# apache/incubator-predictionio

Measured on AMD Instinct MI355X. Metric: als_ratings_per_sec, higher is better.
Workload: dtype fp32; 1 GPU; model=als_rank64_implicit, global_batch=250000000, users=12500000, items=10000000, parallelism=dp1

## Files before the change

### predictionio_amd/ops/csrc/als_kernels.hip

```cpp

#include <hip/hip_runtime.h>

#define CHUNK 16

__device__ __forceinline__ void wave_sync() {
  __builtin_amdgcn_wave_barrier();
}

typedef __attribute__((ext_vector_type(4))) float f32x4_t;
typedef __attribute__((ext_vector_type(2))) float f32x2_t;
typedef __attribute__((ext_vector_type(16))) float f32x16_t;

__device__ __forceinline__ f32x2_t fma2(f32x2_t a, f32x2_t b, f32x2_t c) {
  return __builtin_elementwise_fma(a, b, c);
}

__device__ __forceinline__ int uniform_i32(int v) {
  return __builtin_amdgcn_readfirstlane(v);
}
__device__ __forceinline__ long long uniform_i64(long long v) {
  const unsigned int lo = (unsigned int)uniform_i32((int)(unsigned long long)v);
  const unsigned int hi =
      (unsigned int)uniform_i32((int)((unsigned long long)v >> 32));
  return (long long)(((unsigned long long)hi << 32) | lo);
}
__device__ __forceinline__ float lane_bcast(float v, int k) {
  return __int_as_float(__builtin_amdgcn_readlane(__float_as_int(v), k));
}


template <int F>
__global__ __launch_bounds__(256) void als_solve_kernel(
    const long long* __restrict__ indptr,
    const int* __restrict__ indices,
    const float* __restrict__ values,
    const float* __restrict__ Y,
    const float* __restrict__ YtY,
    float* __restrict__ X,
    int n_rows,
    float lambda,
    float alpha,
    int implicit_mode,
    int wr_scale,
    int skip_below)
{
  constexpr int TM = 4;
  constexpr int TILES = (F / TM) * (F / TM);
  constexpr int TPT = (TILES + 255) / 256;
  constexpr int NB = 16;
  static_assert(F % TM == 0, "F must be divisible by 4");
  static_assert(F % NB == 0, "F must be divisible by the panel width");

  __shared__ float ys[CHUNK][F + 1];
  __shared__ float ws_a[CHUNK];
  __shared__ float ws_b[CHUNK];
  __shared__ float As[F][F + 4];
  __shared__ float bs[F];
  __shared__ float dinv_all[F];

  const int tid = threadIdx.x;
  const int lane = tid & 63;
  const int wave = tid >> 6;

  for (long long row = blockIdx.x; row < n_rows; row += gridDim.x) {
    const long long start = indptr[row];
    const long long end = indptr[row + 1];
    const int nnz = (int)(end - start);
    if (nnz <= skip_below) continue;

    float acc[TPT][TM][TM];
#pragma unroll
    for (int t = 0; t < TPT; ++t)
#pragma unroll
      for (int i = 0; i < TM; ++i)
#pragma unroll
        for (int j = 0; j < TM; ++j) acc[t][i][j] = 0.f;

    for (int i = tid; i < F; i += 256) bs[i] = 0.f;

    for (int base = 0; base < nnz; base += CHUNK) {
      const int cn = min(CHUNK, nnz - base);
      __syncthreads();
      for (int e = tid; e < cn * F; e += 256) {
        const int c = e / F;
        const int k = e % F;
        const int col = indices[start + base + c];
        ys[c][k] = Y[(long long)col * F + k];
      }
      if (tid < cn) {
        const float r = values[start + base + tid];
        if (implicit_mode) {
          ws_a[tid] = alpha * r;
          ws_b[tid] = 1.f + alpha * r;
        } else {
          ws_a[tid] = 1.f;
          ws_b[tid] = r;
        }
      }
      __syncthreads();

      if (tid < F) {
        float bacc = 0.f;
        for (int c = 0; c < cn; ++c) bacc += ws_b[c] * ys[c][tid];
        bs[tid] += bacc;
      }

#pragma unroll
      for (int t = 0; t < TPT; ++t) {
        const int tile = tid + t * 256;
        if (TILES >= 256 || tile < TILES) {
          const int ti = (tile / (F / TM)) * TM;
          const int tj = (tile % (F / TM)) * TM;
          for (int c = 0; c < cn; ++c) {
            const float w = ws_a[c];
            float ya[TM], yb[TM];
#pragma unroll
            for (int i = 0; i < TM; ++i) ya[i] = ys[c][ti + i];
#pragma unroll
            for (int j = 0; j < TM; ++j) yb[j] = ys[c][tj + j];
#pragma unroll
            for (int i = 0; i < TM; ++i)
#pragma unroll
              for (int j = 0; j < TM; ++j)
                acc[t][i][j] = fmaf(w * ya[i], yb[j], acc[t][i][j]);
          }
        }
      }
    }
    __syncthreads();

#pragma unroll
    for (int t = 0; t < TPT; ++t) {
      const int tile = tid + t * 256;
      if (TILES >= 256 || tile < TILES) {
        const int ti = (tile / (F / TM)) * TM;
        const int tj = (tile % (F / TM)) * TM;
#pragma unroll
        for (int i = 0; i < TM; ++i)
#pragma unroll
          for (int j = 0; j < TM; ++j) {
            float v = acc[t][i][j];
            if (YtY != nullptr) v += YtY[(ti + i) * F + (tj + j)];
            As[ti + i][tj + j] = v;
          }
      }
    }
    __syncthreads();
    if (tid < F) {
      const float reg = wr_scale ? lambda * (float)nnz : lambda;
      As[tid][tid] += reg;
    }
    __syncthreads();

    for (int k0 = 0; k0 < F; k0 += NB) {
      if (wave == 0) {
        for (int kk = 0; kk < NB; ++kk) {
          const int kq = k0 + kk;
          wave_sync();
          float d = As[kq][kq];
          d = d > 0.f ? sqrtf(d) : 1e-20f;
          const float dinv = 1.f / d;
          if (lane == kk) {
            As[kq][kq] = d;
            dinv_all[kq] = dinv;
          }
          if (lane > kk && lane < NB) As[k0 + lane][kq] *= dinv;
          wave_sync();
          if (lane > kk && lane < NB) {
            const float lik = As[k0 + lane][kq];
            for (int j = kk + 1; j <= lane; ++j)
              As[k0 + lane][k0 + j] =
                  fmaf(-lik, As[k0 + j][kq], As[k0 + lane][k0 + j]);
          }
        }
      }
      __syncthreads();
      if (k0 + NB >= F) break;
      for (int i = k0 + NB + tid; i < F; i += 256) {
        float w[NB];
#pragma unroll
        for (int m = 0; m < NB; ++m) w[m] = As[i][k0 + m];
#pragma unroll
        for (int j = 0; j < NB; ++j) {
          float s = w[j];
#pragma unroll
          for (int m = 0; m < NB; ++m)
            if (m < j) s = fmaf(-w[m], As[k0 + j][k0 + m], s);
          w[j] = s * dinv_all[k0 + j];
        }
#pragma unroll
        for (int m = 0; m < NB; ++m) As[i][k0 + m] = w[m];
      }
      __syncthreads();
      const int rem = F - k0 - NB;
      const int remt = rem >> 1;
      for (int e = tid; e < remt * remt; e += 256) {
        const int i = k0 + NB + 2 * (e / remt);
        const int j = k0 + NB + 2 * (e % remt);
        if (j <= i) {
          float s00 = As[i][j];
          float s01 = As[i][j + 1];
          float s10 = As[i + 1][j];
          float s11 = As[i + 1][j + 1];
#pragma unroll
          for (int m = 0; m < NB; m += 4) {
            const f32x4_t a0 =
                *reinterpret_cast<const f32x4_t*>(&As[i][k0 + m]);
            const f32x4_t a1 =
                *reinterpret_cast<const f32x4_t*>(&As[i + 1][k0 + m]);
            const f32x4_t b0 =
                *reinterpret_cast<const f32x4_t*>(&As[j][k0 + m]);
            const f32x4_t b1 =
                *reinterpret_cast<const f32x4_t*>(&As[j + 1][k0 + m]);
#pragma unroll
            for (int q = 0; q < 4; ++q) {
              s00 = fmaf(-a0[q], b0[q], s00);
              s01 = fmaf(-a0[q], b1[q], s01);
              s10 = fmaf(-a1[q], b0[q], s10);
              s11 = fmaf(-a1[q], b1[q], s11);
            }
          }
          As[i][j] = s00;
          if (j + 1 <= i) As[i][j + 1] = s01;
          As[i + 1][j] = s10;
          As[i + 1][j + 1] = s11;
        }
      }
      __syncthreads();
    }

    for (int k0 = 0; k0 < F; k0 += NB) {
      if (wave == 0) {
        for (int kk = 0; kk < NB; ++kk) {
          wave_sync();
          const float zk = bs[k0 + kk] * dinv_all[k0 + kk];
          if (lane == kk) bs[k0 + kk] = zk;
          if (lane > kk && lane < NB)
            bs[k0 + lane] = fmaf(-As[k0 + lane][k0 + kk], zk,
                                 bs[k0 + lane]);
        }
      }
      __syncthreads();
      for (int j = k0 + NB + tid; j < F; j += 256) {
        float s = bs[j];
#pragma unroll
        for (int m = 0; m < NB; ++m)
          s = fmaf(-As[j][k0 + m], bs[k0 + m], s);
        bs[j] = s;
      }
      __syncthreads();
    }
    for (int k0 = F - NB; k0 >= 0; k0 -= NB) {
      if (wave == 0) {
        for (int kk = NB - 1; kk >= 0; --kk) {
          wave_sync();
          const float xk = bs[k0 + kk] * dinv_all[k0 + kk];
          if (lane == kk) bs[k0 + kk] = xk;
          if (lane < kk)
            bs[k0 + lane] = fmaf(-As[k0 + kk][k0 + lane], xk,
                                 bs[k0 + lane]);
        }
      }
      __syncthreads();
      for (int j = tid; j < k0; j += 256) {
        float s = bs[j];
#pragma unroll
        for (int m = 0; m < NB; ++m)
          s = fmaf(-As[k0 + m][j], bs[k0 + m], s);
        bs[j] = s;
      }
      __syncthreads();
    }

    if (tid < F) X[row * (long long)F + tid] = bs[tid];
    __syncthreads();
  }
}


constexpr int wave_kernel_min_waves(int f) {
  return f <= 16 ? 6 : (f <= 32 ? 4 : 2);
}

template <int F, bool BF16G = false>
__global__ __launch_bounds__(128, wave_kernel_min_waves(F))
void als_solve_wave_kernel(
    const long long* __restrict__ indptr,
    const int* __restrict__ indices,
    const float* __restrict__ values,
    const float* __restrict__ Y,
    const float* __restrict__ YtY,
    float* __restrict__ X,
    int n_rows,
    float lambda,
    float alpha,
    int implicit_mode,
    int wr_scale,
    int skip_below,
    int skip_above)
{
  static_assert(F <= 64, "wave kernel supports rank <= 64");
  static_assert(!BF16G || F == 64, "MFMA Gramian variant needs F=64");
  const int lane = threadIdx.x & 63;
  const int wave = uniform_i32((int)(threadIdx.x >> 6));

  constexpr int PD = 4;
  constexpr int LP = F + 4;
  __shared__ float ys[2][PD][F];
  constexpr int TP = 40;
  __shared__ unsigned short ysT[2][BF16G ? F : 1][BF16G ? TP : 1];
  __shared__ float Lc[2][F][LP];

  for (long long row = (long long)blockIdx.x * 2 + wave; row < n_rows;
       row += (long long)gridDim.x * 2) {
    const long long start = uniform_i64(indptr[row]);
    const int nnz = uniform_i32((int)(indptr[row + 1] - start));
    if (nnz <= skip_below || nnz > skip_above)
      continue;

    const int ln = lane | (int)(start >> 63);

    f32x2_t ap[F / 2];
#pragma unroll
    for (int m = 0; m < F / 2; ++m) ap[m] = f32x2_t{0.f, 0.f};
    float b_reg = 0.f;

    if constexpr (BF16G) {
      typedef __attribute__((ext_vector_type(8))) unsigned short bf16x8g;
      typedef __attribute__((ext_vector_type(4))) float f32x4g;
      const int lg = lane >> 4;
      const int lq = lane & 15;
      f32x4g accm[4][4];
#pragma unroll
      for (int ti = 0; ti < 4; ++ti)
#pragma unroll
        for (int tj = 0; tj < 4; ++tj)
          accm[ti][tj] = f32x4g{0.f, 0.f, 0.f, 0.f};
      float yn2[PD], wa2[PD], wb2[PD];
#pragma unroll
      for (int p = 0; p < PD; ++p) {
        if (p < nnz) {
          const int col = indices[start + p];
          yn2[p] = lane < F ? Y[(long long)col * F + lane] : 0.f;
          const float v = values[start + p];
          wa2[p] = implicit_mode ? alpha * v : 1.f;
          wb2[p] = implicit_mode ? 1.f + alpha * v : v;
        }
      }
      for (int c0 = 0; c0 < nnz; c0 += 32) {
        for (int cm = 0; cm < 32; ++cm) {
          const int c = c0 + cm;
          const int slot = c & (PD - 1);
          float sy = 0.f;
          if (c < nnz) {
            const float wa = wa2[slot];
            const float sc = sqrtf(wa > 1e-12f ? wa : 1e-12f);
            const float ycur = yn2[slot];
            sy = sc * ycur;
            b_reg = fmaf(wb2[slot], ycur, b_reg);
            if (c + PD < nnz) {
              const int ncol = indices[start + c + PD];
              yn2[slot] = lane < F ? Y[(long long)ncol * F + lane] : 0.f;
              const float nv = values[start + c + PD];
              wa2[slot] = implicit_mode ? alpha * nv : 1.f;
              wb2[slot] = implicit_mode ? 1.f + alpha * nv : nv;
            }
          }
          const unsigned short hb =
              (unsigned short)(__float_as_uint(sy) >> 16);
          const int gcol = (((cm >> 3) ^ (lane & 3)) << 3) | (cm & 7);
          ysT[wave][lane][gcol] = hb;
        }
        wave_sync();
        bf16x8g frag[4];
#pragma unroll
        for (int t = 0; t < 4; ++t) {
          const int row = t * 16 + lq;
          const int g = lg ^ (row & 3);
          frag[t] = *reinterpret_cast<const bf16x8g*>(
              &ysT[wave][row][g << 3]);
        }
#pragma unroll
        for (int ti = 0; ti < 4; ++ti)
#pragma unroll
          for (int tj = 0; tj < 4; ++tj)
            accm[ti][tj] = __builtin_amdgcn_mfma_f32_16x16x32_bf16(
                frag[ti], frag[tj], accm[ti][tj], 0, 0, 0);
        wave_sync();
      }
#pragma unroll
      for (int ti = 0; ti < 4; ++ti)
#pragma unroll
        for (int tj = 0; tj < 4; ++tj)
#pragma unroll
          for (int r = 0; r < 4; ++r)
            Lc[wave][ti * 16 + lg * 4 + r][tj * 16 + lq] =
                accm[ti][tj][r];
      wave_sync();
#pragma unroll
      for (int m = 0; m < F; ++m) ap[m >> 1][m & 1] = Lc[wave][m][lane];
      wave_sync();
    } else {
    float yn[PD], vn[PD];
#pragma unroll
    for (int p = 0; p < PD; ++p) {
      if (p < nnz) {
        const int col = indices[start + p];
        yn[p] = lane < F ? Y[(long long)col * F + lane] : 0.f;
        vn[p] = values[start + p];
      }
    }
    for (int c0 = 0; c0 < nnz; c0 += PD) {
#pragma unroll
      for (int p = 0; p < PD; ++p) {
        const int c = c0 + p;
        if (c >= nnz) break;
        const float ycur = yn[p];
        const float vcur = vn[p];
        if (lane < F) ys[wave][p][lane] = ycur;
        wave_sync();
        if (c + PD < nnz) {
          const int ncol = indices[start + c + PD];
          if (lane < F) yn[p] = Y[(long long)ncol * F + lane];
          vn[p] = values[start + c + PD];
        }
        float w_a, w_b;
        if (implicit_mode) {
          w_a = alpha * vcur;
          w_b = 1.f + alpha * vcur;
        } else {
          w_a = 1.f;
          w_b = vcur;
        }
        b_reg = fmaf(w_b, ycur, b_reg);
        const float wyj = w_a * ycur;
        const f32x2_t wyj2 = {wyj, wyj};
#pragma unroll
        for (int q = 0; q < F / 4; ++q) {
          const f32x4_t y4 =
              *reinterpret_cast<const f32x4_t*>(&ys[wave][p][4 * q]);
          ap[2 * q + 0] = fma2(wyj2, y4.lo, ap[2 * q + 0]);
          ap[2 * q + 1] = fma2(wyj2, y4.hi, ap[2 * q + 1]);
        }
        wave_sync();
      }
    }

    }

    if (YtY != nullptr && lane < F) {
#pragma unroll
      for (int q = 0; q < F / 4; ++q) {
        const f32x4_t t4 = *reinterpret_cast<const f32x4_t*>(
            &YtY[(long long)lane * F + 4 * q]);
        ap[2 * q + 0] += t4.lo;
        ap[2 * q + 1] += t4.hi;
      }
    }
    {
      const float reg = wr_scale ? lambda * (float)nnz : lambda;
#pragma unroll
      for (int m = 0; m < F; ++m)
        if (m == ln) ap[m >> 1][m & 1] += reg;
    }

    float dl = 0.f;
#pragma unroll
    for (int k = 0; k < F; ++k) {
      float lkk = lane_bcast(ap[k >> 1][k & 1], k);
      lkk = lkk > 1e-30f ? lkk : 1e-30f;
      const float dinv = rsqrtf(lkk);
      const float ljk = ln > k ? ap[k >> 1][k & 1] * dinv : 0.f;
      dl = ln == k ? dinv : dl;
      Lc[wave][k][lane < F ? lane : F] = ljk;
      ap[k >> 1][k & 1] = ljk;
      wave_sync();
      const f32x2_t nl2 = {-ljk, -ljk};
#pragma unroll
      for (int m4 = (k + 1) & ~3; m4 < F; m4 += 4) {
        const f32x4_t lq =
            *reinterpret_cast<const f32x4_t*>(&Lc[wave][k][m4]);
        const f32x2_t lh[2] = {lq.lo, lq.hi};
#pragma unroll
        for (int h = 0; h < 2; ++h) {
          const int m2 = m4 + 2 * h;
          if (m2 > k)
            ap[m2 >> 1] = fma2(nl2, lh[h], ap[m2 >> 1]);
          else if (m2 == k)
            ap[m2 >> 1][1] = fmaf(-ljk, lh[h][1], ap[m2 >> 1][1]);
        }
      }
      wave_sync();
    }

#pragma unroll
    for (int k = 0; k < F; ++k) {
      const float zk = lane_bcast(b_reg * dl, k);
      b_reg = fmaf(-ap[k >> 1][k & 1], zk, b_reg);
    }
    b_reg *= dl;
    {
      float4 lq = {0.f, 0.f, 0.f, 0.f};
#pragma unroll
      for (int k = F - 1; k >= 0; --k) {
        if ((k & 3) == 3 && lane < F)
          lq = *reinterpret_cast<const float4*>(&Lc[wave][lane][k & ~3]);
        const float xk = lane_bcast(b_reg * dl, k);
        const float lv = (k & 3) == 0 ? lq.x
                         : (k & 3) == 1 ? lq.y
                         : (k & 3) == 2 ? lq.z : lq.w;
        b_reg = fmaf(ln < k ? -lv : 0.f, xk, b_reg);
      }
      b_reg *= dl;
    }

    if (lane < F) X[row * (long long)F + lane] = b_reg;
  }
}


#define WOODBURY_MAX_NNZ 32


template <int F, int NW, int NLO, bool BF16S = false>
__global__ __launch_bounds__(128, NW > 24 ? 5 : 6) void als_woodbury_kernel(
    const long long* __restrict__ indptr,
    const int* __restrict__ indices,
    const float* __restrict__ values,
    const float* __restrict__ Y,
    const float* __restrict__ V,
    float* __restrict__ X,
    int n_rows,
    float lambda,
    float alpha,
    int implicit_mode,
    int wr_scale,
    unsigned long long* prof)
{
  constexpr int FP = F + 4;
  constexpr int FPH = F + 8;
  const int lane = threadIdx.x & 63;
  const int wave = uniform_i32((int)(threadIdx.x >> 6));

  __shared__ float Yl[2][NW][BF16S ? (FPH / 2) : FP];
  constexpr int MP = NW + 4;
  __shared__ float M[2][NW][MP];
  __shared__ float tv[2][NW];
  __shared__ __attribute__((aligned(16)))
  float dv[2][NW];

  float* yl = &Yl[wave][0][0];
  unsigned short* ylh = reinterpret_cast<unsigned short*>(yl);
  const float* src = implicit_mode ? V : Y;
  const unsigned short* srch = reinterpret_cast<const unsigned short*>(V);

  for (long long row = (long long)blockIdx.x * 2 + wave; row < n_rows;
       row += (long long)gridDim.x * 2) {
    const long long start = uniform_i64(indptr[row]);
    const int n = uniform_i32((int)(indptr[row + 1] - start));
    if (n > NW || n <= NLO) continue;
    if (n == 0 && NLO < 0) {
      for (int e = lane; e < F; e += 64)
        X[row * (long long)F + e] = 0.f;
      continue;
    }
    const bool probe = prof != nullptr && (row & 1023) == 0 && lane == 0;
    unsigned long long pt0 = 0, pt1 = 0, pt2 = 0, pt3 = 0;
    if (probe) pt0 = wall_clock64();

    if (lane < n)
      tv[wave][lane] = __int_as_float(indices[start + lane]);
    wave_sync();
    for (int c = 0; c < n; ++c) {
      const long long col = __float_as_int(tv[wave][c]);
      if constexpr (BF16S) {
        const unsigned int* srow = reinterpret_cast<const unsigned int*>(
            srch + col * F);
        unsigned int* drow =
            reinterpret_cast<unsigned int*>(ylh + c * FPH);
        for (int e = lane; e < F / 2; e += 64) drow[e] = srow[e];
      } else {
        for (int e = lane; e < F; e += 64)
          yl[c * FP + e] = src[col * F + e];
      }
    }
    if (lane < n) {
      const float r = values[start + lane];
      if (implicit_mode) {
        const float ar = alpha * r;
        const float d = sqrtf(ar > 1e-12f ? ar : 1e-12f);
        dv[wave][lane] = d;
        tv[wave][lane] = (1.f + ar) / d;
      } else {
        tv[wave][lane] = r;
      }
    }
    wave_sync();
    if (probe) pt1 = wall_clock64();

    const float reg = wr_scale ? lambda * (float)n : lambda;
    constexpr bool MFMA_G = !BF16S && NW >= 24;
    if constexpr (MFMA_G) {
      const int gj = lane & 31, gh = lane >> 5;
      const f32x4_t* vq = reinterpret_cast<const f32x4_t*>(
          &yl[(gj < NW ? gj : NW - 1) * FP + 4 * gh]);
      f32x16_t acc = {0.f, 0.f, 0.f, 0.f, 0.f, 0.f, 0.f, 0.f,
                      0.f, 0.f, 0.f, 0.f, 0.f, 0.f, 0.f, 0.f};
#pragma unroll
      for (int q = 0; q < F / 8; ++q) {
        const f32x4_t a = vq[2 * q];
        acc = __builtin_amdgcn_mfma_f32_32x32x2f32(a.x, a.x, acc, 0, 0, 0);
        acc = __builtin_amdgcn_mfma_f32_32x32x2f32(a.y, a.y, acc, 0, 0, 0);
        acc = __builtin_amdgcn_mfma_f32_32x32x2f32(a.z, a.z, acc, 0, 0, 0);
        acc = __builtin_amdgcn_mfma_f32_32x32x2f32(a.w, a.w, acc, 0, 0, 0);
      }
      static_assert(NW % 4 == 0 && NW <= 32, "one 32x32 tile, whole quads");
      const float dj = dv[wave][gj < NW ? gj : NW - 1];
      const float dg = implicit_mode ? 1.f : reg;
      f32x4_t dadd;
#pragma unroll
      for (int t = 0; t < 4; ++t) dadd[t] = (gj & 3) == t ? dg : 0.f;
#pragma unroll
      for (int b = 0; b < (NW + 7) / 8; ++b) {
        const int c0 = 8 * b + 4 * gh;
        if (gj < NW && c0 < NW) {
          const f32x4_t d4 = *reinterpret_cast<const f32x4_t*>(&dv[wave][c0]);
          const bool diag = (gj >> 2) == 2 * b + gh;
          f32x4_t m4;
#pragma unroll
          for (int t = 0; t < 4; ++t) {
            const float sc = implicit_mode ? dj * d4[t] : 1.f;
            m4[t] = acc[4 * b + t] * sc + (diag ? dadd[t] : 0.f);
          }
          *reinterpret_cast<f32x4_t*>(&M[wave][gj][c0]) = m4;
        }
      }
    } else {
      const int npairs = n * (n + 1) / 2;
      int p = lane, i = 0;
      while (p >= n - i && i < n) { p -= n - i; ++i; }
      int j = i + p;
      for (int pp = lane; pp < npairs; pp += 64) {
        float dot;
        if constexpr (BF16S) {
          const uint4* yi8 = reinterpret_cast<const uint4*>(&ylh[i * FPH]);
          const uint4* yj8 = reinterpret_cast<const uint4*>(&ylh[j * FPH]);
          f32x4_t acc4 = {0.f, 0.f, 0.f, 0.f};
#pragma unroll
          for (int q = 0; q < F / 8; ++q) {
            const uint4 a = yi8[q];
            const uint4 b = yj8[q];
            const unsigned int av[4] = {a.x, a.y, a.z, a.w};
            const unsigned int bv[4] = {b.x, b.y, b.z, b.w};
#pragma unroll
            for (int t = 0; t < 4; ++t) {
              acc4.x = fmaf(__uint_as_float(av[t] << 16),
                            __uint_as_float(bv[t] << 16), acc4.x);
              acc4.y = fmaf(__uint_as_float(av[t] & 0xffff0000u),
                            __uint_as_float(bv[t] & 0xffff0000u), acc4.y);
            }
          }
          dot = acc4.x + acc4.y;
        } else {
          const f32x4_t* yi = reinterpret_cast<const f32x4_t*>(&yl[i * FP]);
          const f32x4_t* yj = reinterpret_cast<const f32x4_t*>(&yl[j * FP]);
          f32x4_t acc4 = {0.f, 0.f, 0.f, 0.f};
#pragma unroll
          for (int q = 0; q < F / 4; ++q) acc4 += yi[q] * yj[q];
          dot = acc4.x + acc4.y + acc4.z + acc4.w;
        }
        if (implicit_mode) {
          dot *= dv[wave][i] * dv[wave][j];
          if (i == j) dot += 1.f;
        } else if (i == j) {
          dot += reg;
        }
        M[wave][i][j] = dot;
        M[wave][j][i] = dot;
        j += 64;
        while (j >= n && i < n) { ++i; j -= n - i; }
      }
    }
    wave_sync();

    if (probe) pt2 = wall_clock64();
    const int ln = lane | (int)(start >> 63);
    f32x2_t mp[NW / 2];
    const float* mrow = &M[wave][lane < NW ? lane : NW - 1][0];
    const int wcol = lane < NW ? lane : NW;
#pragma unroll
    for (int q = 0; q < NW / 4; ++q) {
      const f32x4_t r4 = *reinterpret_cast<const f32x4_t*>(&mrow[4 * q]);
      mp[2 * q + 0] = lane < n ? r4.lo : f32x2_t{0.f, 0.f};
      mp[2 * q + 1] = lane < n ? r4.hi : f32x2_t{0.f, 0.f};
    }
    float t = lane < n ? tv[wave][lane] : 0.f;
    float dl = 0.f;
    wave_sync();
#pragma unroll
    for (int k = 0; k < NW; ++k) {
      if (k < n) {
        float mkk = lane_bcast(mp[k >> 1][k & 1], k);
        mkk = mkk > 1e-30f ? mkk : 1e-30f;
        const float dinv = rsqrtf(mkk);
        const float ljk = ln > k ? mp[k >> 1][k & 1] * dinv : 0.f;
        dl = ln == k ? dinv : dl;
        mp[k >> 1][k & 1] = ljk;
        M[wave][k][wcol] = ljk;
        wave_sync();
        const f32x2_t nl2 = {-ljk, -ljk};
#pragma unroll
        for (int j4 = (k + 1) & ~3; j4 < NW; j4 += 4) {
          const f32x4_t q4 =
              *reinterpret_cast<const f32x4_t*>(&M[wave][k][j4]);
          const f32x2_t qh[2] = {q4.lo, q4.hi};
#pragma unroll
          for (int h = 0; h < 2; ++h) {
            const int j2 = j4 + 2 * h;
            if (j2 > k)
              mp[j2 >> 1] = fma2(nl2, qh[h], mp[j2 >> 1]);
            else if (j2 == k)
              mp[j2 >> 1][1] = fmaf(-ljk, qh[h][1], mp[j2 >> 1][1]);
          }
        }
        wave_sync();
      }
    }
#pragma unroll
    for (int k = 0; k < NW; ++k) {
      if (k < n) {
        const float zk = lane_bcast(t * dl, k);
        t = fmaf(-mp[k >> 1][k & 1], zk, t);
      }
    }
    t *= dl;
    wave_sync();
#pragma unroll
    for (int q = 0; q < NW / 4; ++q) {
      const f32x4_t r4 = *reinterpret_cast<const f32x4_t*>(&mrow[4 * q]);
      mp[2 * q + 0] = r4.lo;
      mp[2 * q + 1] = r4.hi;
    }
#pragma unroll
    for (int k = NW - 1; k >= 0; --k) {
      if (k < n) {
        const float xk = lane_bcast(t * dl, k);
        t = fmaf(ln < k ? -mp[k >> 1][k & 1] : 0.f, xk, t);
      }
    }
    t *= dl;
    if (implicit_mode) t *= dv[wave][lane < n ? lane : 0];
    if (lane < n) tv[wave][lane] = t;
    wave_sync();

    if (probe) pt3 = wall_clock64();
    for (int e = lane; e < F; e += 64) {
      float x = 0.f;
      for (int c = 0; c < n; ++c) {
        float ye;
        if constexpr (BF16S)
          ye = __uint_as_float((unsigned int)ylh[c * FPH + e] << 16);
        else
          ye = yl[c * FP + e];
        x = fmaf(tv[wave][c], ye, x);
      }
      X[row * (long long)F + e] = x;
    }
    if (probe) {
      const unsigned long long pt4 = wall_clock64();
      atomicAdd(&prof[0], pt1 - pt0);
      atomicAdd(&prof[1], pt2 - pt1);
      atomicAdd(&prof[2], pt3 - pt2);
      atomicAdd(&prof[3], pt4 - pt3);
      atomicAdd(&prof[4], 1ull);
    }
    wave_sync();
  }
}


template <int F, int NW, int NLO, bool BF16S = false>
__global__ __launch_bounds__(128, 3) void als_woodbury2_kernel(
    const long long* __restrict__ indptr,
    const int* __restrict__ indices,
    const float* __restrict__ values,
    const float* __restrict__ Y,
    const float* __restrict__ V,
    float* __restrict__ X,
    int n_rows,
    float lambda,
    float alpha,
    int implicit_mode,
    int wr_scale,
    unsigned long long* prof)
{
  constexpr int FP = F + 4;
  constexpr int FPH = F + 8;
  constexpr int MP = NW + 4;
  const int lane = threadIdx.x & 63;
  const int wave = threadIdx.x >> 6;
  const int h = lane >> 5;
  const int r = lane & 31;

  __shared__ float Yl[2][2][NW][BF16S ? (FPH / 2) : FP];
  constexpr int YROW = BF16S ? (FPH / 2) : FP;
  __shared__ float M[2][2][NW][MP];
  __shared__ float tv[2][2][NW];
  __shared__ float dv[2][2][NW];

  const float* src = implicit_mode ? V : Y;
  const unsigned short* srch = reinterpret_cast<const unsigned short*>(V);

  for (long long base = ((long long)blockIdx.x * 2 + wave) * 2;
       base < n_rows; base += (long long)gridDim.x * 4) {
    int nh[2];
    long long starth[2];
    bool act[2];
#pragma unroll
    for (int hh = 0; hh < 2; ++hh) {
      const long long row = base + hh;
      if (row < n_rows) {
        starth[hh] = indptr[row];
        nh[hh] = (int)(indptr[row + 1] - starth[hh]);
        act[hh] = nh[hh] <= NW && nh[hh] > NLO;
        if (nh[hh] == 0 && NLO < 0) {
          for (int e = lane; e < F; e += 64)
            X[row * (long long)F + e] = 0.f;
          act[hh] = false;
        }
      } else {
        act[hh] = false;
        nh[hh] = 0;
        starth[hh] = 0;
      }
    }
    if (!act[0] && !act[1]) continue;
    const bool probe = prof != nullptr && (base & 1023) == 0 && lane == 0
                       && act[0];
    unsigned long long pt0 = 0, pt1 = 0, pt2 = 0, pt3 = 0;
    if (probe) pt0 = wall_clock64();

#pragma unroll
    for (int hh = 0; hh < 2; ++hh) {
      if (!act[hh]) continue;
      const int n = nh[hh];
      const long long start = starth[hh];
      float* yl = &Yl[wave][hh][0][0];
      unsigned short* ylh = reinterpret_cast<unsigned short*>(yl);
      if (lane < n)
        tv[wave][hh][lane] = __int_as_float(indices[start + lane]);
      wave_sync();
      for (int c = 0; c < n; ++c) {
        const long long col = __float_as_int(tv[wave][hh][c]);
        if constexpr (BF16S) {
          const unsigned int* srow = reinterpret_cast<const unsigned int*>(
              srch + col * F);
          unsigned int* drow =
              reinterpret_cast<unsigned int*>(ylh + c * FPH);
          for (int e = lane; e < F / 2; e += 64) drow[e] = srow[e];
        } else {
          for (int e = lane; e < F; e += 64)
            yl[c * FP + e] = src[col * F + e];
        }
      }
      if (lane < n) {
        const float v = values[start + lane];
        if (implicit_mode) {
          const float ar = alpha * v;
          const float d = sqrtf(ar > 1e-12f ? ar : 1e-12f);
          dv[wave][hh][lane] = d;
          tv[wave][hh][lane] = (1.f + ar) / d;
        } else {
          tv[wave][hh][lane] = v;
        }
      }
    }
    wave_sync();
    if (probe) pt1 = wall_clock64();

    const int n = nh[h];
    {
      const float* yl = &Yl[wave][h][0][0];
      const unsigned short* ylh =
          reinterpret_cast<const unsigned short*>(yl);
      const float reg = wr_scale ? lambda * (float)n : lambda;
      const int npairs = act[h] ? n * (n + 1) / 2 : 0;
      int p = r, i = 0;
      while (p >= n - i && i < n) { p -= n - i; ++i; }
      int j = i + p;
      for (int pp = r; pp < npairs; pp += 32) {
        float dot;
        if constexpr (BF16S) {
          const uint4* yi8 = reinterpret_cast<const uint4*>(&ylh[i * FPH]);
          const uint4* yj8 = reinterpret_cast<const uint4*>(&ylh[j * FPH]);
          f32x4_t acc4 = {0.f, 0.f, 0.f, 0.f};
#pragma unroll
          for (int q = 0; q < F / 8; ++q) {
            const uint4 a = yi8[q];
            const uint4 b = yj8[q];
            const unsigned int av[4] = {a.x, a.y, a.z, a.w};
            const unsigned int bv[4] = {b.x, b.y, b.z, b.w};
#pragma unroll
            for (int t = 0; t < 4; ++t) {
              acc4.x = fmaf(__uint_as_float(av[t] << 16),
                            __uint_as_float(bv[t] << 16), acc4.x);
              acc4.y = fmaf(__uint_as_float(av[t] & 0xffff0000u),
                            __uint_as_float(bv[t] & 0xffff0000u), acc4.y);
            }
          }
          dot = acc4.x + acc4.y;
        } else {
          const f32x4_t* yi = reinterpret_cast<const f32x4_t*>(&yl[i * FP]);
          const f32x4_t* yj = reinterpret_cast<const f32x4_t*>(&yl[j * FP]);
          f32x4_t acc4 = {0.f, 0.f, 0.f, 0.f};
#pragma unroll
          for (int q = 0; q < F / 4; ++q) acc4 += yi[q] * yj[q];
          dot = acc4.x + acc4.y + acc4.z + acc4.w;
        }
        if (implicit_mode) {
          dot *= dv[wave][h][i] * dv[wave][h][j];
          if (i == j) dot += 1.f;
        } else if (i == j) {
          dot += reg;
        }
        M[wave][h][i][j] = dot;
        M[wave][h][j][i] = dot;
        j += 32;
        while (j >= n && i < n) { ++i; j -= n - i; }
      }
    }
    wave_sync();
    if (probe) pt2 = wall_clock64();

    float mr[NW];
#pragma unroll
    for (int q = 0; q < NW; ++q)
      mr[q] = (r < n && q < n) ? M[wave][h][r][q] : 0.f;
    float t = r < n ? tv[wave][h][r] : 0.f;
    wave_sync();
    const int hb = lane & 32;
#pragma unroll
    for (int k = 0; k < NW; ++k) {
      if (k < n) {
        float mkk = __shfl(mr[k], hb + k);
        mkk = mkk > 1e-30f ? mkk : 1e-30f;
        const float dinv = rsqrtf(mkk);
        const float ljk = r > k ? mr[k] * dinv
                                : (r == k ? mkk * dinv : 0.f);
        mr[k] = ljk;
        if (r < NW) M[wave][h][k][r] = ljk;
      }
      wave_sync();
      if (k < n) {
#pragma unroll
        for (int j4 = (k + 1) & ~3; j4 < NW; j4 += 4) {
          if (j4 < n) {
            const float4 q4 =
                *reinterpret_cast<const float4*>(&M[wave][h][k][j4]);
            if (r > k) {
              if (j4 + 0 > k) mr[j4 + 0] = fmaf(-mr[k], q4.x, mr[j4 + 0]);
              if (j4 + 1 > k) mr[j4 + 1] = fmaf(-mr[k], q4.y, mr[j4 + 1]);
              if (j4 + 2 > k) mr[j4 + 2] = fmaf(-mr[k], q4.z, mr[j4 + 2]);
              if (j4 + 3 > k) mr[j4 + 3] = fmaf(-mr[k], q4.w, mr[j4 + 3]);
            }
          }
        }
      }
      wave_sync();
    }
#pragma unroll
    for (int k = 0; k < NW; ++k) {
      if (k < n) {
        const float lkk = __shfl(mr[k], hb + k);
        const float zk = __shfl(t, hb + k) / lkk;
        if (r == k) t = zk;
        else if (r > k) t = fmaf(-mr[k], zk, t);
      }
    }
    wave_sync();
#pragma unroll
    for (int k = NW - 1; k >= 0; --k) {
      if (k < n) {
        const float lkk = __shfl(mr[k], hb + k);
        const float xk = __shfl(t, hb + k) / lkk;
        if (r == k) t = xk;
        else if (r < k) t = fmaf(-M[wave][h][r][k], xk, t);
      }
    }
    if (implicit_mode) t *= dv[wave][h][r < n ? r : 0];
    if (r < n && act[h]) tv[wave][h][r] = t;
    wave_sync();
    if (probe) pt3 = wall_clock64();

#pragma unroll
    for (int hh = 0; hh < 2; ++hh) {
      if (!act[hh]) continue;
      const float* yl = &Yl[wave][hh][0][0];
      const unsigned short* ylh =
          reinterpret_cast<const unsigned short*>(yl);
      const int nn = nh[hh];
      const long long row = base + hh;
      for (int e = lane; e < F; e += 64) {
        float x = 0.f;
        for (int c = 0; c < nn; ++c) {
          float ye;
          if constexpr (BF16S)
            ye = __uint_as_float(
                (unsigned int)ylh[c * FPH + e] << 16);
          else
            ye = yl[c * FP + e];
          x = fmaf(tv[wave][hh][c], ye, x);
        }
        X[row * (long long)F + e] = x;
      }
    }
    if (probe) {
      const unsigned long long pt4 = wall_clock64();
      atomicAdd(&prof[0], pt1 - pt0);
      atomicAdd(&prof[1], pt2 - pt1);
      atomicAdd(&prof[2], pt3 - pt2);
      atomicAdd(&prof[3], pt4 - pt3);
      atomicAdd(&prof[4], 1ull);
    }
    wave_sync();
  }
}



template <int FF>
static void launch_wave_bf16g(int grid_w, hipStream_t stream,
    const long long* indptr, const int* indices, const float* values,
    const float* Y, const float* YtY, float* X, int n_rows, float lambda,
    float alpha, int implicit_mode, int wr_scale, int skip, int wave_hi) {
  if constexpr (FF == 64) {
    hipLaunchKernelGGL((als_solve_wave_kernel<64, true>), dim3(grid_w),
                       dim3(128), 0, stream, indptr, indices, values, Y,
                       YtY, X, n_rows, lambda, alpha, implicit_mode,
                       wr_scale, skip, wave_hi);
  }
}

extern "C" void launch_als_solve(
    const long long* indptr, const int* indices, const float* values,
    const float* Y, const float* YtY, const float* V, float* X,
    int n_rows, int f, float lambda, float alpha,
    int implicit_mode, int wr_scale, int which,
    unsigned long long* prof, hipStream_t stream)
{
  if (n_rows <= 0) return;
  long long wg = ((long long)n_rows + 1) / 2;
  int grid_w = (int)(wg < (1 << 20) ? wg : (1 << 20));
  int grid_b = n_rows < (1 << 20) ? n_rows : (1 << 20);
  const bool woodbury = which != 2 &&
      (implicit_mode ? V != nullptr : true);
  const int skip = (woodbury || which == 2) ? WOODBURY_MAX_NNZ : -1;
  const bool dense = which != 1;
  const char* e_split = getenv("PIO_ALS_DENSE_SPLIT");
  const int dense_split = e_split ? atoi(e_split) : 0;
  const int wave_hi = dense_split > 0 ? dense_split : 0x7fffffff;
#define LAUNCH_WAVE(FF)                                                      \
  if (dense && use_bf16s_g && FF == 64) {                                    \
  launch_wave_bf16g<FF>(grid_w, stream, indptr, indices, values, Y, YtY, X, \
                        n_rows, lambda, alpha, implicit_mode, wr_scale,      \
                        skip, wave_hi);                                      \
  if (dense_split > 0)                                                       \
    hipLaunchKernelGGL((als_solve_kernel<FF>), dim3(grid_b), dim3(256), 0,   \
                       stream, indptr, indices, values, Y, YtY, X, n_rows,   \
                       lambda, alpha, implicit_mode, wr_scale, dense_split); \
  } else if (dense) {                                                        \
  hipLaunchKernelGGL((als_solve_wave_kernel<FF>), dim3(grid_w), dim3(128),   \
                     0, stream, indptr, indices, values, Y, YtY, X, n_rows,  \
                     lambda, alpha, implicit_mode, wr_scale, skip, wave_hi); \
  if (dense_split > 0)                                                       \
    hipLaunchKernelGGL((als_solve_kernel<FF>), dim3(grid_b), dim3(256), 0,   \
                       stream, indptr, indices, values, Y, YtY, X, n_rows,   \
                       lambda, alpha, implicit_mode, wr_scale, dense_split); \
  }
#define LAUNCH_BLOCK(FF)                                                     \
  if (dense)                                                                 \
  hipLaunchKernelGGL((als_solve_kernel<FF>), dim3(grid_b), dim3(256), 0,     \
                     stream, indptr, indices, values, Y, YtY, X, n_rows,     \
                     lambda, alpha, implicit_mode, wr_scale, skip)
  const char* e_dual = getenv("PIO_ALS_DUAL");
  const bool use_dual = e_dual != nullptr && e_dual[0] == '1';
  const char* e_bf16 = getenv("PIO_ALS_STAGE_BF16");
  const bool stage_bf16 = e_bf16 != nullptr && e_bf16[0] == '1';
  const bool use_bf16s = stage_bf16 && implicit_mode && V != nullptr;
  const char* e_mg = getenv("PIO_ALS_MFMA_GRAMIAN");
  const bool use_bf16s_g = e_mg != nullptr && e_mg[0] == '1';
  long long wg4 = ((long long)n_rows + 3) / 4;
  int grid_w2 = (int)(wg4 < (1 << 20) ? wg4 : (1 << 20));
#define LAUNCH_WOODBURY(FF)                                                  \
  if (woodbury && use_dual && use_bf16s) {                                   \
    hipLaunchKernelGGL((als_woodbury2_kernel<FF, 20, -1, true>),             \
                       dim3(grid_w2), dim3(128), 0, stream, indptr,          \
                       indices, values, Y, V, X, n_rows, lambda, alpha,      \
                       implicit_mode, wr_scale, prof);                       \
    hipLaunchKernelGGL((als_woodbury2_kernel<FF, 24, 20, true>),             \
                       dim3(grid_w2), dim3(128), 0, stream, indptr,          \
                       indices, values, Y, V, X, n_rows, lambda, alpha,      \
                       implicit_mode, wr_scale, prof);                       \
    hipLaunchKernelGGL((als_woodbury_kernel<FF, 32, 24, true>),              \
                       dim3(grid_w), dim3(128), 0, stream, indptr, indices,  \
                       values, Y, V, X, n_rows, lambda, alpha,               \
                       implicit_mode, wr_scale, prof);                       \
  } else if (woodbury && use_dual) {                                         \
      \
      \
      \
    hipLaunchKernelGGL((als_woodbury2_kernel<FF, 20, -1>), dim3(grid_w2),    \
                       dim3(128), 0, stream, indptr, indices, values, Y, V,  \
                       X, n_rows, lambda, alpha, implicit_mode, wr_scale,    \
                       prof);                                                \
    hipLaunchKernelGGL((als_woodbury2_kernel<FF, 24, 20>), dim3(grid_w2),    \
                       dim3(128), 0, stream, indptr, indices, values, Y, V,  \
                       X, n_rows, lambda, alpha, implicit_mode, wr_scale,    \
                       prof);                                                \
    hipLaunchKernelGGL((als_woodbury_kernel<FF, 32, 24>), dim3(grid_w),      \
                       dim3(128), 0, stream, indptr, indices, values, Y, V,  \
                       X, n_rows, lambda, alpha, implicit_mode, wr_scale,    \
                       prof);                                                \
  } else if (woodbury && use_bf16s) {                                        \
    hipLaunchKernelGGL((als_woodbury_kernel<FF, 20, -1, true>),              \
                       dim3(grid_w), dim3(128), 0, stream, indptr, indices,  \
                       values, Y, V, X, n_rows, lambda, alpha,               \
                       implicit_mode, wr_scale, prof);                       \
    hipLaunchKernelGGL((als_woodbury_kernel<FF, 24, 20, true>),              \
                       dim3(grid_w), dim3(128), 0, stream, indptr, indices,  \
                       values, Y, V, X, n_rows, lambda, alpha,               \
                       implicit_mode, wr_scale, prof);                       \
    hipLaunchKernelGGL((als_woodbury_kernel<FF, 32, 24, true>),              \
                       dim3(grid_w), dim3(128), 0, stream, indptr, indices,  \
                       values, Y, V, X, n_rows, lambda, alpha,               \
                       implicit_mode, wr_scale, prof);                       \
  } else if (woodbury) {                                                     \
    hipLaunchKernelGGL((als_woodbury_kernel<FF, 20, -1>), dim3(grid_w),      \
                       dim3(128), 0, stream, indptr, indices, values, Y, V,  \
                       X, n_rows, lambda, alpha, implicit_mode, wr_scale,    \
                       prof);                                                \
    hipLaunchKernelGGL((als_woodbury_kernel<FF, 24, 20>), dim3(grid_w),      \
                       dim3(128), 0, stream, indptr, indices, values, Y, V,  \
                       X, n_rows, lambda, alpha, implicit_mode, wr_scale,    \
                       prof);                                                \
    hipLaunchKernelGGL((als_woodbury_kernel<FF, 32, 24>), dim3(grid_w),      \
                       dim3(128), 0, stream, indptr, indices, values, Y, V,  \
                       X, n_rows, lambda, alpha, implicit_mode, wr_scale,    \
                       prof);                                                \
  }
  switch (f) {
    case 16: LAUNCH_WOODBURY(16); LAUNCH_WAVE(16); break;
    case 32: LAUNCH_WOODBURY(32); LAUNCH_WAVE(32); break;
    case 64: LAUNCH_WOODBURY(64); LAUNCH_WAVE(64); break;
    case 128: LAUNCH_WOODBURY(128); LAUNCH_BLOCK(128); break;
    default: break;
  }
#undef LAUNCH_WAVE
#undef LAUNCH_BLOCK
#undef LAUNCH_WOODBURY
}
```

Before: 1.922 billion ratings/s.

## Ballot-compact row ownership and extend Woodbury path to 48 nnz with MFMA Gramian

Each wave now takes a 64-row tile, reads every row's degree in parallel and ballots a mask of the rows that fall in its nnz bucket, then loops only over those rows. Before, each kernel strode over every row and skipped most of them one at a time. The Woodbury low-rank solve also gains two new buckets (33-40 and 41-48 nnz) for rank 64/128. Their Gramian is built from 16x16x4 MFMA blocks, which moves rows out of the heavier dense Cholesky wave kernel. The cost is more shared memory and registers per wave in the wide buckets (min waves drops to 2), plus an extra indptr scan in every kernel.

Measured after the change: 2.189 billion ratings/s (median of 6 runs). 13.8% higher.

```diff
diff --git a/predictionio_amd/ops/csrc/als_kernels.hip b/predictionio_amd/ops/csrc/als_kernels.hip
--- a/predictionio_amd/ops/csrc/als_kernels.hip
+++ b/predictionio_amd/ops/csrc/als_kernels.hip
@@ -26,6 +26,16 @@
 }
 __device__ __forceinline__ float lane_bcast(float v, int k) {
   return __int_as_float(__builtin_amdgcn_readlane(__float_as_int(v), k));
+}
+
+__device__ __forceinline__ unsigned long long owned_rows_mask(
+    const long long* __restrict__ indptr, long long base, int n_rows,
+    int lane, int lo, int hi) {
+  const long long r = base + lane;
+  const long long r0 = r < n_rows ? r : n_rows;
+  const long long r1 = r + 1 < n_rows ? r + 1 : n_rows;
+  const int deg = (int)(indptr[r1] - indptr[r0]);
+  return __builtin_amdgcn_ballot_w64(r < n_rows && deg > lo && deg <= hi);
 }
 
 
@@ -311,12 +321,15 @@
   __shared__ unsigned short ysT[2][BF16G ? F : 1][BF16G ? TP : 1];
   __shared__ float Lc[2][F][LP];
 
-  for (long long row = (long long)blockIdx.x * 2 + wave; row < n_rows;
-       row += (long long)gridDim.x * 2) {
+  for (long long base = ((long long)blockIdx.x * 2 + wave) * 64;
+       base < n_rows; base += (long long)gridDim.x * 128) {
+    unsigned long long todo =
+        owned_rows_mask(indptr, base, n_rows, lane, skip_below, skip_above);
+  while (todo != 0) {
+    const long long row = base + __builtin_ctzll(todo);
+    todo &= todo - 1;
     const long long start = uniform_i64(indptr[row]);
     const int nnz = uniform_i32((int)(indptr[row + 1] - start));
-    if (nnz <= skip_below || nnz > skip_above)
-      continue;
 
     const int ln = lane | (int)(start >> 63);
 
@@ -516,14 +529,23 @@
 
     if (lane < F) X[row * (long long)F + lane] = b_reg;
   }
-}
-
-
-#define WOODBURY_MAX_NNZ 32
-
+  }
+}
+
+
+
+constexpr int woodbury_min_waves(int nw) {
+  return nw > 32 ? 2 : (nw > 24 ? 5 : 6);
+}
+#ifdef PIO_ALS_WIDE_G_VALU
+constexpr bool WIDE_G_ON_MFMA = false;
+#else
+constexpr bool WIDE_G_ON_MFMA = true;
+#endif
 
 template <int F, int NW, int NLO, bool BF16S = false>
-__global__ __launch_bounds__(128, NW > 24 ? 5 : 6) void als_woodbury_kernel(
+__global__ __launch_bounds__(128, woodbury_min_waves(NW))
+void als_woodbury_kernel(
     const long long* __restrict__ indptr,
     const int* __restrict__ indices,
     const float* __restrict__ values,
@@ -554,8 +576,13 @@
   const float* src = implicit_mode ? V : Y;
   const unsigned short* srch = reinterpret_cast<const unsigned short*>(V);
 
-  for (long long row = (long long)blockIdx.x * 2 + wave; row < n_rows;
-       row += (long long)gridDim.x * 2) {
+  for (long long base = ((long long)blockIdx.x * 2 + wave) * 64;
+       base < n_rows; base += (long long)gridDim.x * 128) {
+    unsigned long long todo =
+        owned_rows_mask(indptr, base, n_rows, lane, NLO, NW);
+  while (todo != 0) {
+    const long long row = base + __builtin_ctzll(todo);
+    todo &= todo - 1;
     const long long start = uniform_i64(indptr[row]);
     const int n = uniform_i32((int)(indptr[row + 1] - start));
     if (n > NW || n <= NLO) continue;
@@ -599,8 +626,65 @@
     if (probe) pt1 = wall_clock64();
 
     const float reg = wr_scale ? lambda * (float)n : lambda;
-    constexpr bool MFMA_G = !BF16S && NW >= 24;
-    if constexpr (MFMA_G) {
+    constexpr bool MFMA_G = !BF16S && NW >= 24 && NW <= 32;
+    constexpr bool MFMA_G16 = !BF16S && NW > 32 && WIDE_G_ON_MFMA;
+    if constexpr (MFMA_G16) {
+      static_assert(NW % 4 == 0 && NW <= 48 && F % 16 == 0,
+                    "3 x 3 blocks of 16, whole quads");
+      const int gr = lane & 15, gk = lane >> 4;
+      const f32x4_t* vq[3];
+#pragma unroll
+      for (int b = 0; b < 3; ++b) {
+        const int r = 16 * b + gr;
+        vq[b] = reinterpret_cast<const f32x4_t*>(
+            &yl[(r < NW ? r : NW - 1) * FP + 4 * gk]);
+      }
+      f32x4_t acc[6];
+#pragma unroll
+      for (int p = 0; p < 6; ++p) acc[p] = f32x4_t{0.f, 0.f, 0.f, 0.f};
+#pragma unroll
+      for (int q = 0; q < F / 16; ++q) {
+        f32x4_t a[3];
+#pragma unroll
+        for (int b = 0; b < 3; ++b) a[b] = vq[b][4 * q];
+#pragma unroll
+        for (int t = 0; t < 4; ++t)
+#pragma unroll
+          for (int bi = 0; bi < 3; ++bi)
+#pragma unroll
+            for (int bj = 0; bj <= bi; ++bj)
+              acc[bi * (bi + 1) / 2 + bj] =
+                  __builtin_amdgcn_mfma_f32_16x16x4f32(
+                      a[bi][t], a[bj][t], acc[bi * (bi + 1) / 2 + bj],
+                      0, 0, 0);
+      }
+      const float dg = implicit_mode ? 1.f : reg;
+#pragma unroll
+      for (int bi = 0; bi < 3; ++bi) {
+        const int R0 = 16 * bi + 4 * gk;
+        f32x4_t dr = {1.f, 1.f, 1.f, 1.f};
+        if (implicit_mode && R0 < NW)
+          dr = *reinterpret_cast<const f32x4_t*>(&dv[wave][R0]);
+#pragma unroll
+        for (int bj = 0; bj <= bi; ++bj) {
+          const int C = 16 * bj + gr;
+          if (R0 < NW && C < NW) {
+            const float dc = implicit_mode ? dv[wave][C] : 1.f;
+            f32x4_t m4;
+#pragma unroll
+            for (int t = 0; t < 4; ++t) {
+              m4[t] = acc[bi * (bi + 1) / 2 + bj][t] * (dr[t] * dc);
+              if (bi == bj) m4[t] += (R0 + t == C) ? dg : 0.f;
+            }
+            *reinterpret_cast<f32x4_t*>(&M[wave][C][R0]) = m4;
+            if (bi != bj) {
+#pragma unroll
+              for (int t = 0; t < 4; ++t) M[wave][R0 + t][C] = m4[t];
+            }
+          }
+        }
+      }
+    } else if constexpr (MFMA_G) {
       const int gj = lane & 31, gh = lane >> 5;
       const f32x4_t* vq = reinterpret_cast<const f32x4_t*>(
           &yl[(gj < NW ? gj : NW - 1) * FP + 4 * gh]);
@@ -775,6 +859,7 @@
       atomicAdd(&prof[4], 1ull);
     }
     wave_sync();
+  }
   }
 }
 
@@ -1028,6 +1113,30 @@
 
 
 
+static int woodbury_max_nnz(int f, bool opt_in) {
+  if ((f != 64 && f != 128) || opt_in) return 32;
+  const char* e = getenv("PIO_ALS_WOODBURY_MAX");
+  if (e != nullptr && e[0] == '3' && e[1] == '2' && e[2] == '\0') return 32;
+  return 48;
+}
+
+template <int FF>
+static void launch_woodbury_wide(int grid_w, hipStream_t stream,
+    const long long* indptr, const int* indices, const float* values,
+    const float* Y, const float* V, float* X, int n_rows, float lambda,
+    float alpha, int implicit_mode, int wr_scale, unsigned long long* prof) {
+  if constexpr (FF >= 64) {
+    hipLaunchKernelGGL((als_woodbury_kernel<FF, 40, 32>), dim3(grid_w),
+                       dim3(128), 0, stream, indptr, indices, values, Y, V,
+                       X, n_rows, lambda, alpha, implicit_mode, wr_scale,
+                       prof);
+    hipLaunchKernelGGL((als_woodbury_kernel<FF, 48, 40>), dim3(grid_w),
+                       dim3(128), 0, stream, indptr, indices, values, Y, V,
+                       X, n_rows, lambda, alpha, implicit_mode, wr_scale,
+                       prof);
+  }
+}
+
 template <int FF>
 static void launch_wave_bf16g(int grid_w, hipStream_t stream,
     const long long* indptr, const int* indices, const float* values,
@@ -1049,12 +1158,11 @@
     unsigned long long* prof, hipStream_t stream)
 {
   if (n_rows <= 0) return;
-  long long wg = ((long long)n_rows + 1) / 2;
+  long long wg = ((long long)n_rows + 127) / 128;
   int grid_w = (int)(wg < (1 << 20) ? wg : (1 << 20));
   int grid_b = n_rows < (1 << 20) ? n_rows : (1 << 20);
   const bool woodbury = which != 2 &&
       (implicit_mode ? V != nullptr : true);
-  const int skip = (woodbury || which == 2) ? WOODBURY_MAX_NNZ : -1;
   const bool dense = which != 1;
   const char* e_split = getenv("PIO_ALS_DENSE_SPLIT");
   const int dense_split = e_split ? atoi(e_split) : 0;
@@ -1089,6 +1197,10 @@
   const bool use_bf16s = stage_bf16 && implicit_mode && V != nullptr;
   const char* e_mg = getenv("PIO_ALS_MFMA_GRAMIAN");
   const bool use_bf16s_g = e_mg != nullptr && e_mg[0] == '1';
+  const int wmax = woodbury_max_nnz(
+      f, use_dual || (stage_bf16 && implicit_mode) ||
+             (use_bf16s_g && f == 64));
+  const int skip = (woodbury || which == 2) ? wmax : -1;
   long long wg4 = ((long long)n_rows + 3) / 4;
   int grid_w2 = (int)(wg4 < (1 << 20) ? wg4 : (1 << 20));
 #define LAUNCH_WOODBURY(FF)                                                  \
@@ -1147,6 +1259,10 @@
                        dim3(128), 0, stream, indptr, indices, values, Y, V,  \
                        X, n_rows, lambda, alpha, implicit_mode, wr_scale,    \
                        prof);                                                \
+    if (wmax > 32)                                                           \
+      launch_woodbury_wide<FF>(grid_w, stream, indptr, indices, values, Y,   \
+                               V, X, n_rows, lambda, alpha, implicit_mode,   \
+                               wr_scale, prof);                              \
   }
   switch (f) {
     case 16: LAUNCH_WOODBURY(16); LAUNCH_WAVE(16); break;
```
